# hiropppe/RocAlphaGo

Measured on AMD Instinct MI355X. Metric: positions/sec SL-policy train + MCTS sims/sec (19x19) at 1/2/4/8 MI355X, higher is better.
Workload: dtype bf16; 1 GPU; global_batch=256, per_gpu_batch=256, seq_len=361, parallelism=dp1

## Files before the change

### csrc/hip/conv_wino.hip

```cpp
#include <atomic>

#include "common.h"
#include "conv_host.h"
#include "pack.h"
#include "rag_api.h"

using namespace rag;

namespace {

constexpr int kWK = 32;
constexpr int kWP = 192;
constexpr int kVRows = 224;
constexpr int kRRows = 512;
constexpr int kVSlot = kVRows * kWK;
constexpr int kLoopLds = 4 * kVSlot;
constexpr int kRedU = 14;

template <int WN, int PAIRS> struct WinoGeo;
template <> struct WinoGeo<192, 192> {
  static constexpr int MW = 2, MT = 6, NT = 3, RG = 2;
};
template <> struct WinoGeo<128, 192> {
  static constexpr int MW = 4, MT = 3, NT = 4, RG = 1;
};
template <> struct WinoGeo<192, 96> {
  static constexpr int MW = 2, MT = 3, NT = 3, RG = 1;
};
template <int WN, int PAIRS> struct WinoTile : WinoGeo<WN, PAIRS> {
  using G = WinoGeo<WN, PAIRS>;
  static_assert(G::MW * 16 * G::MT == PAIRS && (8 / G::MW) * 16 * G::NT == WN, "wave tiling");
  static constexpr int EpRow = WN + 8;
  static constexpr int EpImg = 2 * PAIRS * EpRow;
  static constexpr int Lds = kLoopLds > EpImg ? kLoopLds : EpImg;
  static_assert(Lds * 2 <= 160 * 1024, "LDS budget");
};
constexpr int kHalfPairs = 96;

__device__ __forceinline__ int swz4w(int row) { return ((row >> 2) & 1) << 1; }

template <int V> struct IntC {
  static constexpr int value = V;
};

typedef uint32_t u32x4 __attribute__((ext_vector_type(4)));
template <int SGN>
__device__ __forceinline__ bf16x8 vaddsub(const bf16x8& a, const bf16x8& b) {
  const u32x4 ua = __builtin_bit_cast(u32x4, a), ub = __builtin_bit_cast(u32x4, b);
  u32x4 o;
#pragma unroll
  for (int w = 0; w < 4; ++w) {
    const float a0 = __uint_as_float(ua[w] << 16), a1 = __uint_as_float(ua[w] & 0xffff0000u);
    const float b0 = __uint_as_float(ub[w] << 16), b1 = __uint_as_float(ub[w] & 0xffff0000u);
    const bf16x2 r = {(bf16)(SGN > 0 ? a0 + b0 : a0 - b0), (bf16)(SGN > 0 ? a1 + b1 : a1 - b1)};
    o[w] = __builtin_bit_cast(uint32_t, r);
  }
  return __builtin_bit_cast(bf16x8, o);
}
__device__ __forceinline__ bf16x8 vsum(const bf16x8& a, const bf16x8& b) { return vaddsub<1>(a, b); }
__device__ __forceinline__ bf16x8 vdiff(const bf16x8& a, const bf16x8& b) { return vaddsub<-1>(a, b); }
template <int SGN>
__device__ __forceinline__ bf16x8 vaddsub_bn(const bf16x8& a, const bf16x8& b, float cxa,
                                             float cca, float cxb, float ccb) {
  const u32x4 ua = __builtin_bit_cast(u32x4, a), ub = __builtin_bit_cast(u32x4, b);
  u32x4 o;
#pragma unroll
  for (int w = 0; w < 4; ++w) {
    const float a0 = fmaxf(fmaf(cxa, __uint_as_float(ua[w] << 16), cca), 0.f);
    const float a1 = fmaxf(fmaf(cxa, __uint_as_float(ua[w] & 0xffff0000u), cca), 0.f);
    const float b0 = fmaxf(fmaf(cxb, __uint_as_float(ub[w] << 16), ccb), 0.f);
    const float b1 = fmaxf(fmaf(cxb, __uint_as_float(ub[w] & 0xffff0000u), ccb), 0.f);
    const bf16x2 r = {(bf16)(SGN > 0 ? a0 + b0 : a0 - b0), (bf16)(SGN > 0 ? a1 + b1 : a1 - b1)};
    o[w] = __builtin_bit_cast(uint32_t, r);
  }
  return __builtin_bit_cast(bf16x8, o);
}

struct WinoBN {
  const float* coef;
  const bf16* res;
  float* spart;
  const float* smean;
};

template <bool SINGLE, int MT> struct WinoGeom {
  int lane, wm, wn, frow, fq;
  int TJ, PB, RPB;
  int b0, n0, p0;
  long total_rows;
  int vb[SINGLE ? 1 : MT];
  uint32_t uoff;
  int tu0, tu1;
};

__device__ __forceinline__ auto wino_rsrc(const void* p, long bytes) {
  const uint64_t a = reinterpret_cast<uint64_t>(p);
  const uint32_t lo = __builtin_amdgcn_readfirstlane((uint32_t)a);
  const uint32_t hi = __builtin_amdgcn_readfirstlane((uint32_t)(a >> 32));
  const int nb = __builtin_amdgcn_readfirstlane((int)(bytes < 0x7fffffffL ? bytes : 0x7fffffffL));
  return __builtin_amdgcn_make_buffer_rsrc(reinterpret_cast<void*>(((uint64_t)hi << 32) | lo),
                                           (short)0, nb, 0x00020000);
}

template <typename R>
__device__ __forceinline__ uint32_t wino_warm(const R& urs, int NOUT, int KIN) {
  uint32_t warm = 0;
  const int lin = blockIdx.y * gridDim.x + blockIdx.x;
  const int per_xcd = (gridDim.x * gridDim.y + 7) >> 3;
  const uint32_t slice = (uint32_t)((12L * NOUT * KIN * 2 + per_xcd - 1) / per_xcd);
  const uint32_t base = (uint32_t)((lin >> 3) % per_xcd) * slice;
#pragma unroll
  for (int k = 0; k < 4; ++k) {
    const uint32_t off = (uint32_t)(threadIdx.x + k * 512) * 16u;
    const uint32_t o = off < slice ? base + off : 0xfffffff0u;
    warm ^= (uint32_t)__builtin_amdgcn_raw_buffer_load_b32(urs, o, 0, 0);
  }
  return warm;
}

template <int WN, bool SINGLE, int PAIRS>
__device__ __forceinline__ WinoGeom<SINGLE, WinoTile<WN, PAIRS>::MT> wino_geom(int B, int S,
                                                                              int nb) {
  using T = WinoTile<WN, PAIRS>;
  constexpr int kWMT = T::MT;
  constexpr bool HALF = PAIRS == kHalfPairs;
  static_assert(!HALF || SINGLE, "half-board blocks: one board");
  WinoGeom<SINGLE, kWMT> g;
  const int lane = lane_id();
  const int w = wave_id();
  g.lane = lane;
  g.wm = w % T::MW;
  g.wn = w / T::MW;
  g.frow = lane & 15;
  g.fq = lane >> 4;
  const int WI = S + 2, TJ = (S + 1) >> 1;
  const int PB = S * TJ;
  const int VPB = WI * TJ;
  const int RPB = WI * WI;
  g.TJ = TJ;
  g.PB = PB;
  g.RPB = RPB;
  g.b0 = HALF ? (int)(blockIdx.x >> 1) : (int)blockIdx.x * nb;
  g.n0 = blockIdx.y * WN;
  const int p0 = HALF ? (int)(blockIdx.x & 1) * kHalfPairs : 0;
  const int i0 = HALF ? p0 / TJ : 0;
  const int voff = p0 - i0 * TJ;
  g.p0 = p0;
  g.total_rows = (long)B * RPB;
#pragma unroll
  for (int i = 0; i < (SINGLE ? 1 : kWMT); ++i) {
    int m = g.wm * (16 * kWMT) + i * 16 + g.frow;
    if (SINGLE) {
      g.vb[i] = m + voff;
      continue;
    }
    m = m < nb * PB ? m : nb * PB - 1;
    const int bl = m / PB, rem = m - bl * PB;
    const int ii = rem / TJ, t = rem - ii * TJ;
    g.vb[i] = (bl * WI + ii) * TJ + t;
  }
  g.uoff = (uint32_t)((((g.n0 >> 4) + g.wn * T::NT) * 512 + lane * 8) * 2);
  const int NU = HALF ? ((p0 + kHalfPairs - 1) / TJ - i0 + 3) * TJ * 4 : nb * VPB * 4;
  auto unit = [&](int it) {
    const int u = threadIdx.x + it * 512;
    const int v = u >> 2;
    const int bl = v / VPB, rem = v - bl * VPB;
    const int r = rem / TJ, t = rem - r * TJ;
    const int rr = (bl * WI + r + i0) * WI + 2 * t;
    return u < NU ? (v | ((u & 3) << 10) | (rr << 12)) : -1;
  };
  g.tu0 = unit(0);
  g.tu1 = unit(1);
  return g;
}

template <int WN, bool SINGLE, int PAIRS, int BNM, bool CHAIN, typename R>
__device__ __forceinline__ void wino_layer(
    const R& urs, bf16* lds, const WinoGeom<SINGLE, WinoTile<WN, PAIRS>::MT>& g,
    const bf16* __restrict__ X, const float* __restrict__ bias, bf16* __restrict__ Y,
    const bf16* __restrict__ mask, int B, int S, int KIN, int NOUT, int HO, int YC, int relu,
    int HM, int nb, const WinoBN& bn, const bf16* Unext) {
  using T = WinoTile<WN, PAIRS>;
  constexpr int kWMT = T::MT, kWNT = T::NT, kWN = WN, kEpRow = T::EpRow;
  constexpr bool HALF = PAIRS == kHalfPairs;
  static_assert(BNM == 0 || (SINGLE && !HALF && WN == 128), "fused BN: the 128-wide one-board tile");
  static_assert(!CHAIN || (BNM == 0 && !HALF), "chain: plain one- or multi-board blocks");
  float* sred = reinterpret_cast<float*>(lds + T::Lds);
  const int lane = g.lane, wm = g.wm, wn = g.wn, frow = g.frow, fq = g.fq;
  const int TJ = g.TJ, PB = g.PB, RPB = g.RPB, b0 = g.b0, n0 = g.n0, p0 = g.p0;
  const long total_rows = g.total_rows;
  const int tu0 = g.tu0, tu1 = g.tu1;
  const int cchunks = KIN / kWK;
  const int NK = 2 * cchunks;
  int vb[SINGLE ? 1 : kWMT];
#pragma unroll
  for (int i = 0; i < (SINGLE ? 1 : kWMT); ++i) vb[i] = g.vb[i];

  const int NF = NOUT / 16;
  const uint32_t uoff = g.uoff;
  auto wfrag = [&](int tap, int c, int j) {
    const int so = ((tap * cchunks + c) * NF + j) * 1024;
    return __builtin_bit_cast(bf16x8, __builtin_amdgcn_raw_buffer_load_b128(urs, uoff, so, 0));
  };

  float bcx[2][4], bcc[2][4];
  if constexpr (BNM == 1) {
#pragma unroll
    for (int q = 0; q < 2; ++q) {
      const int pk = q ? tu1 : tu0;
      const int v = pk < 0 ? 0 : (pk & 1023);
      const int r = v / TJ, t = v - r * TJ;
      const bool rin = pk >= 0 && r >= 1 && r <= S;
#pragma unroll
      for (int s = 0; s < 4; ++s) {
        const int pc = 2 * t + s;
        const bool in = rin && pc >= 1 && pc <= S;
        bcx[q][s] = in ? bn.coef[pc - 1] : 0.f;
        bcc[q][s] = in ? bn.coef[2 * S + pc - 1] : 0.f;
      }
    }
  }
  const auto xrs = wino_rsrc(X + (long)b0 * RPB * KIN, (total_rows - (long)b0 * RPB) * KIN * 2);
  bf16x8 da0, db0, da1, db1;
  auto op_unit = [&](int o, int& v, int& k8, int& rr) {
    int pk = (o >> 1) ? tu1 : tu0;
    asm volatile("" : "+v"(pk));
    v = pk < 0 ? -1 : (pk & 1023);
    pk = pk < 0 ? 0 : pk;
    k8 = (pk >> 10) & 3;
    rr = pk >> 12;
  };
  auto op_load = [&](auto p1c, int kk, auto oc) {
    constexpr bool P1 = decltype(p1c)::value;
    constexpr int o = decltype(oc)::value, h = o & 1;
    int v, k8, rr;
    op_unit(o, v, k8, rr);
    const int ra = P1 ? 1 : (h ? 3 : 0), rb = P1 ? 2 : (h ? 1 : 2);
    const int so = (kk % cchunks) * kWK * 2;
    const uint32_t o0 = (uint32_t)((rr + ra) * KIN + k8 * 8) * 2u;
    const uint32_t o1 = (uint32_t)((rr + rb) * KIN + k8 * 8) * 2u;
    const bf16x8 a = __builtin_bit_cast(bf16x8, __builtin_amdgcn_raw_buffer_load_b128(xrs, o0, so, 0));
    const bf16x8 b = __builtin_bit_cast(bf16x8, __builtin_amdgcn_raw_buffer_load_b128(xrs, o1, so, 0));
    if constexpr (h) {
      da1 = a;
      db1 = b;
    } else {
      da0 = a;
      db0 = b;
    }
  };
  auto op_store = [&](auto p1c, int kk, auto oc) {
    constexpr bool P1 = decltype(p1c)::value;
    constexpr int o = decltype(oc)::value, h = o & 1;
    int v, k8, rr;
    op_unit(o, v, k8, rr);
    v = v < 0 ? kVRows - 1 : v;
    bf16* vs = lds + (kk & 1) * 2 * kVSlot + h * kVSlot;
    const bf16x8 da = h ? da1 : da0, db = h ? db1 : db0;
    bf16x8 val;
    if constexpr (BNM == 1) {
      constexpr int q = o >> 1, ra = P1 ? 1 : (h ? 3 : 0), rb = P1 ? 2 : (h ? 1 : 2);
      if constexpr (P1 && h)
        val = vaddsub_bn<-1>(db, da, bcx[q][rb], bcc[q][rb], bcx[q][ra], bcc[q][ra]);
      else
        val = vaddsub_bn<P1 ? 1 : -1>(da, db, bcx[q][ra], bcc[q][ra], bcx[q][rb], bcc[q][rb]);
    } else {
      val = P1 ? (h ? vdiff(db, da) : vsum(da, db)) : vdiff(da, db);
    }
    *reinterpret_cast<bf16x8*>(vs + v * kWK + ((k8 ^ swz4w(v)) * 8)) = val;
  };

  f32x4 accA[kWNT][kWMT], accB[kWNT][kWMT];
#pragma unroll
  for (int j = 0; j < kWNT; ++j)
#pragma unroll
    for (int i = 0; i < kWMT; ++i) {
      accA[j][i] = f32x4{0.f, 0.f, 0.f, 0.f};
      accB[j][i] = f32x4{0.f, 0.f, 0.f, 0.f};
    }
  constexpr int kH = kWMT / T::RG;
  bf16x8 xa[kH], wA[kWNT], wB[kWNT];
  auto read_v = [&](int kk, int ky, int set, int h) {
    const bf16* vs = lds + ((kk & 1) * 2 + set) * kVSlot;
    const int sh = ky * TJ;
    if constexpr (SINGLE) {
      int r0 = vb[0];
      asm volatile("" : "+v"(r0));
      r0 += sh + h * kH * 16;
      const int sw0 = (fq ^ swz4w(r0)) * 8;
#pragma unroll
      for (int i = 0; i < kH; ++i)
        xa[i] = *reinterpret_cast<const bf16x8*>(vs + (r0 + i * 16) * kWK + sw0);
    } else {
#pragma unroll
      for (int i = 0; i < kH; ++i) {
        int v = vb[h * kH + i];
        asm volatile("" : "+v"(v));
        const int r = v + sh;
        xa[i] = *reinterpret_cast<const bf16x8*>(vs + r * kWK + ((fq ^ swz4w(r)) * 8));
      }
    }
  };

  uint32_t warm = 0;
  if constexpr (!CHAIN) warm = wino_warm(urs, NOUT, KIN);
#pragma unroll
  for (int j = 0; j < kWNT; ++j) {
    wA[j] = wfrag(1, 0, j);
    wB[j] = wfrag(2, 0, j);
  }
  op_load(IntC<1>{}, 0, IntC<0>{});
  op_store(IntC<1>{}, 0, IntC<0>{});
  op_load(IntC<1>{}, 0, IntC<1>{});
  op_store(IntC<1>{}, 0, IntC<1>{});
  op_load(IntC<1>{}, 0, IntC<2>{});
  op_store(IntC<1>{}, 0, IntC<2>{});
  op_load(IntC<1>{}, 0, IntC<3>{});
  op_store(IntC<1>{}, 0, IntC<3>{});
  if constexpr (!CHAIN) asm volatile("" ::"v"(warm));
  asm volatile("s_waitcnt lgkmcnt(0)" ::: "memory");
  __builtin_amdgcn_s_barrier();
  asm volatile("" ::: "memory");

  auto chunk_phase = [&](int kk, auto curc, auto nxtc) {
    constexpr bool CUR1 = decltype(curc)::value, NXT1 = decltype(nxtc)::value;
#pragma unroll
    for (int ky = 0; ky < 3; ++ky) {
      const bool nxt1 = ky < 2 ? CUR1 : NXT1;
      int nkk = ky < 2 ? kk : kk + 1, nky = ky < 2 ? ky + 1 : 0;
      if (nkk >= NK) {
        nkk = NK - 1;
        nky = 2;
      }
      const int nc = nkk % cchunks;
      const int ntA = nky * 4 + (nxt1 ? 1 : 0), ntB = nky * 4 + (nxt1 ? 2 : 3);
      if (ky == 1) op_store(nxtc, kk + 1, IntC<0>{});
      if (ky == 2) op_store(nxtc, kk + 1, IntC<2>{});
      __builtin_amdgcn_sched_barrier(0);
      if (ky == 0) op_load(nxtc, kk + 1, IntC<0>{});
      if (ky == 1) op_load(nxtc, kk + 1, IntC<2>{});
      __builtin_amdgcn_sched_barrier(0);
#pragma unroll
      for (int h = 0; h < T::RG; ++h) {
        read_v(kk, ky, 0, h);
#pragma unroll
        for (int j = 0; j < kWNT; ++j) {
#pragma unroll
          for (int i = 0; i < kH; ++i)
            accA[j][h * kH + i] = mfma16(wA[j], xa[i], accA[j][h * kH + i]);
          if (h == T::RG - 1) wA[j] = wfrag(ntA, nc, j);
        }
      }
      __builtin_amdgcn_sched_barrier(0);
      if (ky == 1) op_store(nxtc, kk + 1, IntC<1>{});
      if (ky == 2) op_store(nxtc, kk + 1, IntC<3>{});
      __builtin_amdgcn_sched_barrier(0);
      if (ky == 0) op_load(nxtc, kk + 1, IntC<1>{});
      if (ky == 1) op_load(nxtc, kk + 1, IntC<3>{});
      __builtin_amdgcn_sched_barrier(0);
#pragma unroll
      for (int h = 0; h < T::RG; ++h) {
        read_v(kk, ky, 1, h);
#pragma unroll
        for (int j = 0; j < kWNT; ++j) {
#pragma unroll
          for (int i = 0; i < kH; ++i)
            accB[j][h * kH + i] = mfma16(wB[j], xa[i], accB[j][h * kH + i]);
          if (h == T::RG - 1) wB[j] = wfrag(ntB, nc, j);
        }
      }
      __builtin_amdgcn_sched_barrier(0);
    }
    asm volatile("s_waitcnt lgkmcnt(0)" ::: "memory");
    __builtin_amdgcn_s_barrier();
    asm volatile("" ::: "memory");
  };

#pragma unroll 1
  for (int kk = 0; kk < cchunks - 1; ++kk) chunk_phase(kk, IntC<1>{}, IntC<1>{});
  chunk_phase(cchunks - 1, IntC<1>{}, IntC<0>{});
#pragma unroll
  for (int j = 0; j < kWNT; ++j)
#pragma unroll
    for (int i = 0; i < kWMT; ++i) {
      const f32x4 a = accA[j][i], b = accB[j][i];
      accA[j][i] = a + b;
      accB[j][i] = a - b;
    }
#pragma unroll 1
  for (int kk = cchunks; kk < NK; ++kk) chunk_phase(kk, IntC<0>{}, IntC<0>{});

  if constexpr (CHAIN) warm = wino_warm(wino_rsrc(Unext, 12L * NOUT * KIN * 2), NOUT, KIN);
  __syncthreads();
#pragma unroll
  for (int j = 0; j < kWNT; ++j) {
    const int n = wn * (16 * kWNT) + j * 16 + fq * 4;
    float4 bb = {0.f, 0.f, 0.f, 0.f};
    if (bias) bb = *reinterpret_cast<const float4*>(bias + n0 + n);
#pragma unroll
    for (int i = 0; i < kWMT; ++i) {
      const int m = wm * (16 * kWMT) + i * 16 + frow;
      bf16x4 oa, ob;
      const float va[4] = {accA[j][i][0] + bb.x, accA[j][i][1] + bb.y, accA[j][i][2] + bb.z,
                           accA[j][i][3] + bb.w};
      const float vb4[4] = {accB[j][i][0] + bb.x, accB[j][i][1] + bb.y, accB[j][i][2] + bb.z,
                            accB[j][i][3] + bb.w};
#pragma unroll
      for (int r = 0; r < 4; ++r) {
        oa[r] = (bf16)(relu ? fmaxf(va[r], 0.f) : va[r]);
        ob[r] = (bf16)(relu ? fmaxf(vb4[r], 0.f) : vb4[r]);
      }
      *reinterpret_cast<bf16x4*>(lds + (2 * m) * kEpRow + n) = oa;
      *reinterpret_cast<bf16x4*>(lds + (2 * m + 1) * kEpRow + n) = ob;
    }
  }
  if constexpr (CHAIN) asm volatile("" ::"v"(warm));
  __syncthreads();
  if constexpr (BNM != 0) {
    const int S2 = S * S, WO = S + 2 * HO, WMK = S + 2 * HM;
    constexpr int kChunks = kWN / 8;
    const int total = S2 * kChunks, nit = (total + 511) / 512;
    const bool st = bn.spart != nullptr;
    for (int it = 0; it < nit; ++it) {
      const int e = threadIdx.x + it * 512;
      const bool valid = e < total;
      const int pix = valid ? e / kChunks : 0, k8 = (e % kChunks) * 8;
      const int i = pix / S, j = pix - (pix / S) * S;
      float s0 = 0.f, s1 = 0.f;
      if (valid) {
        const int m = i * TJ + (j >> 1);
        bf16x8 v = *reinterpret_cast<const bf16x8*>(lds + (2 * m + (j & 1)) * kEpRow + k8);
        const size_t yo = (size_t)((b0 * WO + i + HO) * WO + j + HO) * YC + n0 + k8;
        if constexpr (BNM == 1) {
          if (bn.res) {
            const bf16x8 r = *reinterpret_cast<const bf16x8*>(bn.res + yo);
#pragma unroll
            for (int q = 0; q < 8; ++q) v[q] = (bf16)((float)v[q] + (float)r[q]);
          }
#pragma unroll
          for (int q = 0; q < 8; ++q) {
            const float f = (float)v[q];
            s0 += f;
            s1 = fmaf(f, f, s1);
          }
        } else {
          const bf16x8 mk = *reinterpret_cast<const bf16x8*>(
              mask + (size_t)((b0 * WMK + i + HM) * WMK + j + HM) * YC + n0 + k8);
          const float cx = bn.coef[j], cc = bn.coef[2 * S + j];
          const float mu = bn.smean ? bn.smean[j] : 0.f;
#pragma unroll
          for (int q = 0; q < 8; ++q) {
            const float xm = (float)mk[q];
            v[q] = fmaf(cx, xm, cc) > 0.f ? v[q] : (bf16)0.f;
            const float d = (float)v[q];
            s0 += d;
            s1 = fmaf(d, xm - mu, s1);
          }
        }
        *reinterpret_cast<bf16x8*>(Y + yo) = v;
      }
      if (st) {
#pragma unroll
        for (int o = kChunks / 2; o > 0; o >>= 1) {
          s0 += __shfl_xor(s0, o, 64);
          s1 += __shfl_xor(s1, o, 64);
        }
        if ((threadIdx.x & (kChunks - 1)) == 0 && valid) {
          atomicAdd(sred + j, s0);
          atomicAdd(sred + 64 + j, s1);
        }
      }
    }
    if (st) {
      __syncthreads();
      if ((int)threadIdx.x < 2 * S) {
        const int q = threadIdx.x / S, c = threadIdx.x - q * S;
        bn.spart[((size_t)blockIdx.x * 2 + q) * S + c] = sred[q * 64 + c];
      }
    }
  } else {
    const int nbl = B - b0 < nb ? B - b0 : nb;
    const int S2 = S * S, WO = S + 2 * HO, WMK = S + 2 * HM;
    constexpr int kChunks = kWN / 8;
    const int pe = p0 + kHalfPairs < PB ? p0 + kHalfPairs : PB;
    const int pixb = HALF ? (p0 / TJ) * S + 2 * (p0 % TJ) : 0;
    const int pixe = HALF ? (pe / TJ) * S + 2 * (pe % TJ) : 0;
    const int total = HALF ? ((pixe < S2 ? pixe : S2) - pixb) * kChunks : nbl * S2 * kChunks;
    for (int e = threadIdx.x; e < total; e += 512) {
      const int pix = e / kChunks + pixb, k8 = (e - (e / kChunks) * kChunks) * 8;
      const int bl = HALF ? 0 : pix / S2, rem = pix - bl * S2;
      const int i = rem / S, j = rem - i * S;
      const int m = bl * PB + i * TJ + (j >> 1) - p0;
      bf16x8 v = *reinterpret_cast<const bf16x8*>(lds + (2 * m + (j & 1)) * kEpRow + k8);
      const int b = b0 + bl;
      if (mask) {
        const bf16x8 mk = *reinterpret_cast<const bf16x8*>(
            mask + (size_t)((b * WMK + i + HM) * WMK + j + HM) * YC + n0 + k8);
#pragma unroll
        for (int q = 0; q < 8; ++q) v[q] = ((float)mk[q] > 0.f) ? v[q] : (bf16)0.f;
      }
      *reinterpret_cast<bf16x8*>(Y + (size_t)((b * WO + i + HO) * WO + j + HO) * YC + n0 + k8) = v;
    }
  }
}

template <int WN, bool SINGLE, int PAIRS = kWP, int BNM = 0>
__global__ void __launch_bounds__(512, 1)
conv_wino_kernel(const bf16* __restrict__ X, const bf16* __restrict__ U,
                 const float* __restrict__ bias, bf16* __restrict__ Y,
                 const bf16* __restrict__ mask, int B, int S, int KIN, int NOUT, int HO, int YC,
                 int relu, int HM, int nb, WgradRed red, WinoBN bn = WinoBN{}) {
  using T = WinoTile<WN, PAIRS>;
  __shared__ __attribute__((aligned(16))) bf16 lds[T::Lds + (BNM ? 256 : 0)];
  if constexpr (BNM != 0) {
    float* sred = reinterpret_cast<float*>(lds + T::Lds);
    if (bn.spart && threadIdx.x < 128) sred[threadIdx.x] = 0.f;
  }
  const auto urs = wino_rsrc(U, 12L * NOUT * KIN * 2);
  const auto g = wino_geom<WN, SINGLE, PAIRS>(B, S, nb);
  wino_layer<WN, SINGLE, PAIRS, BNM, false>(urs, lds, g, X, bias, Y, mask, B, S, KIN, NOUT, HO,
                                            YC, relu, HM, nb, bn, nullptr);
  if (red.ticket) wslab_reduce_dynamic<kRedU>(red, reinterpret_cast<int*>(lds));
}

constexpr int kChainMax = 16;
struct WinoChain {
  bf16* act[kChainMax + 1];
  const bf16* U[kChainMax];
  const float* bias[kChainMax];
  uint32_t relu;
  int L;
};
template <int WN, bool SINGLE>
__global__ void __launch_bounds__(512, 1)
conv_wino_chain_kernel(WinoChain c, int B, int S, int nb) {
  using T = WinoTile<WN, kWP>;
  __shared__ __attribute__((aligned(16))) bf16 lds[T::Lds];
  const auto g = wino_geom<WN, SINGLE, kWP>(B, S, nb);
  const uint32_t warm = wino_warm(wino_rsrc(c.U[0], 12L * WN * WN * 2), WN, WN);
  asm volatile("" ::"v"(warm));
#pragma unroll 1
  for (int l = 0; l < c.L; ++l) {
    const int ln = l + 1 < c.L ? l + 1 : l;
    wino_layer<WN, SINGLE, kWP, 0, true>(wino_rsrc(c.U[l], 12L * WN * WN * 2), lds, g, c.act[l],
                                         c.bias[l], c.act[l + 1], nullptr, B, S, WN, WN, 1, WN,
                                         (int)((c.relu >> l) & 1u), 1, nb, WinoBN{}, c.U[ln]);
    asm volatile("s_waitcnt vmcnt(0) lgkmcnt(0)" ::: "memory");
    __builtin_amdgcn_fence(__ATOMIC_RELEASE, "workgroup");
    __syncthreads();
    __builtin_amdgcn_fence(__ATOMIC_ACQUIRE, "workgroup");
  }
}

__global__ void __launch_bounds__(256) __attribute__((amdgpu_waves_per_eu(4)))
wino_pack_kernel(const int64_t* __restrict__ table, SgdFold sgd) {
  __shared__ float tl[kWinoPackLds];
  wino_pack_block(table, (int)blockIdx.y, (int)blockIdx.x, sgd, tl);
}

struct SgdRest {
  float* p;
  long a0, n0, a1, n1;
};

__global__ void __launch_bounds__(256) __attribute__((amdgpu_waves_per_eu(4)))
pack_step_kernel(const int64_t* __restrict__ wtable, int nwino,
                 const int64_t* __restrict__ ttable, int nrows, int nfull, int max_taps,
                 SgdFold sgd, SgdRest rest) {
  extern __shared__ float lds_dyn[];
  int y = (int)blockIdx.y;
  const int bx = (int)blockIdx.x, gx = (int)gridDim.x;
  const int trows = nfull + (nrows > nfull ? 1 : 0);
  if (y < trows) {
    pack_trunk_block(ttable, y, nrows, nfull, sgd, bx, gx, max_taps, lds_dyn);
    return;
  }
  y -= trows;
  const long n = rest.n0 + rest.n1;
  if (n > 0 && y == 0) {
    for (long i = (long)bx * 256 + threadIdx.x; i < n; i += (long)gx * 256) {
      float* w = rest.p + (i < rest.n0 ? rest.a0 + i : rest.a1 + (i - rest.n0));
      *w = sgd.update(*w, w[sgd.goff]);
    }
    return;
  }
  y -= n > 0 ? 1 : 0;
  if (y < nwino) wino_pack_block(wtable, y, bx, sgd, lds_dyn);
}

int wino_boards_per_block(int S) {
  const int WI = S + 2, TJ = (S + 1) / 2;
  const int PB = S * TJ, VPB = WI * TJ, RPB = WI * WI;
  int nb = kWP / PB;
  if (nb * VPB > kVRows) nb = kVRows / VPB;
  if (nb * RPB + 1 > kRRows) nb = (kRRows - 1) / RPB;
  return nb;
}

int wino_tile(int NOUT, int S) {
  if (NOUT % 192 == 0) return 192;
  if (NOUT == 128 && wino_boards_per_block(S) == 1) return 128;
  return 0;
}

}

RAG_API int rag_conv_wino_ok(int S, int HI, int KIN, int NOUT, int KS) {
  return KS == 3 && HI == 1 && KIN % kWK == 0 && KIN >= kWK && S >= 2 &&
         wino_boards_per_block(S) >= 1 && wino_tile(NOUT, S) > 0;
}

static bool wino_half_ok(int S, int NOUT) {
  const int TJ = (S + 1) / 2;
  return NOUT % 192 == 0 && wino_boards_per_block(S) == 1 && S * TJ > kHalfPairs;
}
static int wino_cus() {
  static std::atomic<int> cus{0};
  int n = cus.load(std::memory_order_relaxed);
  if (!n) {
    int dev = 0;
    if (hipGetDevice(&dev) != hipSuccess ||
        hipDeviceGetAttribute(&n, hipDeviceAttributeMultiprocessorCount, dev) != hipSuccess)
      return 0;
    cus.store(n, std::memory_order_relaxed);
  }
  return n;
}
static int wino_mode(int B, int S, int KIN, int NOUT) {
  if (!rag_conv_wino_ok(S, 1, KIN, NOUT, 3) || B <= 0 || wino_boards_per_block(S) != 1) return 0;
  const int cus = wino_cus();
  if (!cus) return 0;
  auto fills = [&](long blocks) {
    const long waves = (blocks + cus - 1) / cus;
    return blocks * 8 >= waves * cus * 7;
  };
  const long full = (long)B * (NOUT / wino_tile(NOUT, S));
  const bool half = wino_half_ok(S, NOUT);
  if (full <= cus) return half && 2 * full <= cus ? 2 : 1;
  if (fills(full)) return 1;
  if (half && fills(2 * full)) return 2;
  return 0;
}
RAG_API int rag_conv_wino_mode(int B, int S, int KIN, int NOUT) {
  return wino_mode(B, S, KIN, NOUT);
}

int rag_conv_wino_launch(const void* X, const void* W, const float* bias, void* Y,
                         const void* mask, int B, int S, int KIN, int NOUT, int HO, int YC,
                         int relu, int HM, hipStream_t stream, const WgradRed* red, int half) {
  if (!rag_conv_wino_ok(S, 1, KIN, NOUT, 3) || YC < NOUT || B <= 0) return -1;
  const int nb = wino_boards_per_block(S);
  WgradRed r{};
  if (red) r = *red;
  const int wt = wino_tile(NOUT, S);
  const dim3 grid((B + nb - 1) / nb, NOUT / wt);
  if (wt == 192 && ((half && wino_half_ok(S, NOUT)) || wino_mode(B, S, KIN, NOUT) == 2))
    conv_wino_kernel<192, true, kHalfPairs><<<dim3(2 * B, NOUT / wt), 512, 0, stream>>>(
        (const bf16*)X, (const bf16*)W, bias, (bf16*)Y, (const bf16*)mask, B, S, KIN, NOUT, HO,
        YC, relu, HM, 1, r);
  else if (wt == 128)
    conv_wino_kernel<128, true><<<grid, 512, 0, stream>>>((const bf16*)X, (const bf16*)W, bias,
                                                          (bf16*)Y, (const bf16*)mask, B, S, KIN,
                                                          NOUT, HO, YC, relu, HM, nb, r);
  else if (nb == 1)
    conv_wino_kernel<192, true><<<grid, 512, 0, stream>>>((const bf16*)X, (const bf16*)W, bias,
                                                          (bf16*)Y, (const bf16*)mask, B, S, KIN,
                                                          NOUT, HO, YC, relu, HM, nb, r);
  else
    conv_wino_kernel<192, false><<<grid, 512, 0, stream>>>((const bf16*)X, (const bf16*)W, bias,
                                                           (bf16*)Y, (const bf16*)mask, B, S, KIN,
                                                           NOUT, HO, YC, relu, HM, nb, r);
  return (int)hipGetLastError();
}

static bool wino_bn_ok(int B, int S, int KIN, int NOUT) {
  return NOUT == 128 && KIN == 128 && S <= 64 && wino_tile(NOUT, S) == 128 &&
         wino_mode(B, S, KIN, NOUT) == 1;
}
RAG_API int rag_conv_wino_bn_ok(int B, int S, int KIN, int NOUT) {
  return wino_bn_ok(B, S, KIN, NOUT);
}

int rag_conv_wino_bn_launch(const void* X, const void* W, const float* bias, void* Y,
                            const void* mask, const void* res, int B, int S, int KIN, int NOUT,
                            int HO, int YC, int relu, int HM, hipStream_t stream,
                            const WgradRed* red, const float* coef, const float* mcoef,
                            float* spart, const float* smean) {
  if (!wino_bn_ok(B, S, KIN, NOUT) || YC < NOUT || (coef != nullptr) == (mcoef != nullptr) ||
      (mcoef && (!mask || res)) || (smean && !mcoef))
    return -5;
  WgradRed r{};
  if (red) r = *red;
  if (coef)
    conv_wino_kernel<128, true, kWP, 1><<<B, 512, 0, stream>>>(
        (const bf16*)X, (const bf16*)W, bias, (bf16*)Y, nullptr, B, S, KIN, NOUT, HO, YC, relu,
        HM, 1, r, WinoBN{coef, (const bf16*)res, spart, nullptr});
  else
    conv_wino_kernel<128, true, kWP, 2><<<B, 512, 0, stream>>>(
        (const bf16*)X, (const bf16*)W, bias, (bf16*)Y, (const bf16*)mask, B, S, KIN, NOUT, HO,
        YC, relu, HM, 1, r, WinoBN{mcoef, nullptr, spart, smean});
  return (int)hipGetLastError();
}

RAG_API int rag_conv_wino_chain(const int64_t* table, int L, int B, int S, hipStream_t stream,
                                int any_batch) {
  constexpr int kF = 7;
  if (!table || L < 1 || L > kChainMax || B <= 0) return -1;
  const int C = (int)table[5];
  if (!rag_conv_wino_ok(S, 1, C, C, 3) || wino_tile(C, S) != C) return -1;
  if (!any_batch && wino_mode(B, S, C, C) != 1) return -1;
  WinoChain c{};
  c.L = L;
  for (int l = 0; l < L; ++l) {
    const int64_t* r = table + (size_t)l * kF;
    if (r[5] != C || r[6] != C || !r[0] || !r[1] || !r[3]) return -1;
    if (l > 0 && r[0] != table[(size_t)(l - 1) * kF + 3]) return -1;
    c.act[l] = reinterpret_cast<bf16*>(r[0]);
    c.act[l + 1] = reinterpret_cast<bf16*>(r[3]);
    c.U[l] = reinterpret_cast<const bf16*>(r[1]);
    c.bias[l] = reinterpret_cast<const float*>(r[2]);
    if (r[4]) c.relu |= 1u << l;
  }
  const int64_t bytes = (int64_t)B * (S + 2) * (S + 2) * C * 2;
  for (int i = 0; i <= L; ++i)
    for (int j = 0; j < i; ++j) {
      const int64_t d = reinterpret_cast<int64_t>(c.act[i]) - reinterpret_cast<int64_t>(c.act[j]);
      if ((d < 0 ? -d : d) < bytes) return -1;
    }
  const int nb = wino_boards_per_block(S);
  const dim3 grid((B + nb - 1) / nb);
  if (C == 128)
    conv_wino_chain_kernel<128, true><<<grid, 512, 0, stream>>>(c, B, S, nb);
  else if (nb == 1)
    conv_wino_chain_kernel<192, true><<<grid, 512, 0, stream>>>(c, B, S, nb);
  else
    conv_wino_chain_kernel<192, false><<<grid, 512, 0, stream>>>(c, B, S, nb);
  return (int)hipGetLastError();
}

RAG_API int rag_wino_pack(const int64_t* table, int nlayers, int max_tiles, hipStream_t stream,
                          int64_t goff, float lr, float wd, int sgd_on) {
  if (nlayers <= 0 || max_tiles <= 0) return -1;
  const dim3 grid((unsigned)(8 * max_tiles), (unsigned)nlayers);
  wino_pack_kernel<<<grid, 256, 0, stream>>>(table, SgdFold{(long)goff, lr, wd, sgd_on});
  return (int)hipGetLastError();
}

RAG_API int rag_pack_step(const int64_t* wtable, int nwino, const int64_t* ttable, int nrows,
                          int nfull, int max_taps, int width, hipStream_t stream, int64_t goff,
                          float lr, float wd, int sgd_on, float* flat, int64_t a0, int64_t n0,
                          int64_t a1, int64_t n1) {
  if (nwino < 0 || nrows < 0 || nfull < 0 || nfull > nrows || width <= 0 || max_taps < 1 ||
      max_taps > kPTaps || n0 < 0 || n1 < 0 || (nwino > 0 && !wtable) || (nrows > 0 && !ttable))
    return -1;
  const bool rest = sgd_on && n0 + n1 > 0;
  if (rest && !flat) return -1;
  const int trows = nfull + (nrows > nfull ? 1 : 0);
  const int rows = nwino + trows + (rest ? 1 : 0);
  if (rows == 0) return 0;
  const int l1 = kWinoPackLds, l2 = pack_trunk_lds(max_taps);
  const size_t lds = (size_t)(nfull > 0 && l2 > l1 ? l2 : l1) * sizeof(float);
  const SgdRest r{flat, (long)a0, rest ? (long)n0 : 0L, (long)a1, rest ? (long)n1 : 0L};
  pack_step_kernel<<<dim3((unsigned)width, (unsigned)rows), 256, lds, stream>>>(
      wtable, nwino, ttable, nrows, nfull, max_taps, SgdFold{(long)goff, lr, wd, sgd_on}, r);
  return (int)hipGetLastError();
}
```

Baseline: 124,300 positions/s.

## Restructure Winograd input-transform pipeline with XOR-flipped LDS ring and precomputed offsets

Reworks the Winograd conv main loop. Per-unit global and LDS offsets are now computed once in the geometry setup instead of being decoded every chunk, and LDS double-buffering switches to an XOR flip bit rather than kk-based slot arithmetic. The P1 pass computes sum and difference together in one fused helper, so one load pair feeds two stores. Half-board blocks now use a single load unit, and a host check keeps that path only when its unit count fits in 512 threads. This cuts address arithmetic and VALU work in the hot loop, at the cost of more persistent registers and a larger LDS footprint from the flip offset.

Result: faster. 127,500 positions/s, median of 6 (+2.5%).

```diff
diff --git a/csrc/hip/conv_wino.hip b/csrc/hip/conv_wino.hip
--- a/csrc/hip/conv_wino.hip
+++ b/csrc/hip/conv_wino.hip
@@ -14,7 +14,9 @@
 constexpr int kVRows = 224;
 constexpr int kRRows = 512;
 constexpr int kVSlot = kVRows * kWK;
-constexpr int kLoopLds = 4 * kVSlot;
+constexpr int kVFlip = 32768;
+constexpr int kLoopLds = kVFlip / 2 + 2 * kVSlot;
+static_assert(2 * kVSlot * 2 <= kVFlip, "V ring: a buffer below the flip bit");
 constexpr int kRedU = 14;
 
 template <int WN, int PAIRS> struct WinoGeo;
@@ -57,8 +59,21 @@
   }
   return __builtin_bit_cast(bf16x8, o);
 }
-__device__ __forceinline__ bf16x8 vsum(const bf16x8& a, const bf16x8& b) { return vaddsub<1>(a, b); }
 __device__ __forceinline__ bf16x8 vdiff(const bf16x8& a, const bf16x8& b) { return vaddsub<-1>(a, b); }
+__device__ __forceinline__ void vsumdiff(const bf16x8& a, const bf16x8& b, bf16x8& s, bf16x8& d) {
+  const u32x4 ua = __builtin_bit_cast(u32x4, a), ub = __builtin_bit_cast(u32x4, b);
+  u32x4 os, od;
+#pragma unroll
+  for (int w = 0; w < 4; ++w) {
+    const float a0 = __uint_as_float(ua[w] << 16), a1 = __uint_as_float(ua[w] & 0xffff0000u);
+    const float b0 = __uint_as_float(ub[w] << 16), b1 = __uint_as_float(ub[w] & 0xffff0000u);
+    const bf16x2 rs = {(bf16)(a0 + b0), (bf16)(a1 + b1)}, rd = {(bf16)(b0 - a0), (bf16)(b1 - a1)};
+    os[w] = __builtin_bit_cast(uint32_t, rs);
+    od[w] = __builtin_bit_cast(uint32_t, rd);
+  }
+  s = __builtin_bit_cast(bf16x8, os);
+  d = __builtin_bit_cast(bf16x8, od);
+}
 template <int SGN>
 __device__ __forceinline__ bf16x8 vaddsub_bn(const bf16x8& a, const bf16x8& b, float cxa,
                                              float cca, float cxb, float ccb) {
@@ -74,6 +89,24 @@
     o[w] = __builtin_bit_cast(uint32_t, r);
   }
   return __builtin_bit_cast(bf16x8, o);
+}
+
+__device__ __forceinline__ void vsumdiff_bn(const bf16x8& a, const bf16x8& b, float cxa, float cca,
+                                            float cxb, float ccb, bf16x8& s, bf16x8& d) {
+  const u32x4 ua = __builtin_bit_cast(u32x4, a), ub = __builtin_bit_cast(u32x4, b);
+  u32x4 os, od;
+#pragma unroll
+  for (int w = 0; w < 4; ++w) {
+    const float a0 = fmaxf(fmaf(cxa, __uint_as_float(ua[w] << 16), cca), 0.f);
+    const float a1 = fmaxf(fmaf(cxa, __uint_as_float(ua[w] & 0xffff0000u), cca), 0.f);
+    const float b0 = fmaxf(fmaf(cxb, __uint_as_float(ub[w] << 16), ccb), 0.f);
+    const float b1 = fmaxf(fmaf(cxb, __uint_as_float(ub[w] & 0xffff0000u), ccb), 0.f);
+    const bf16x2 rs = {(bf16)(a0 + b0), (bf16)(a1 + b1)}, rd = {(bf16)(b0 - a0), (bf16)(b1 - a1)};
+    os[w] = __builtin_bit_cast(uint32_t, rs);
+    od[w] = __builtin_bit_cast(uint32_t, rd);
+  }
+  s = __builtin_bit_cast(bf16x8, os);
+  d = __builtin_bit_cast(bf16x8, od);
 }
 
 struct WinoBN {
@@ -91,6 +124,9 @@
   int vb[SINGLE ? 1 : MT];
   uint32_t uoff;
   int tu0, tu1;
+  uint32_t ru[2];
+  int su[2];
+  int rv[3];
 };
 
 __device__ __forceinline__ auto wino_rsrc(const void* p, long bytes) {
@@ -120,7 +156,7 @@
 
 template <int WN, bool SINGLE, int PAIRS>
 __device__ __forceinline__ WinoGeom<SINGLE, WinoTile<WN, PAIRS>::MT> wino_geom(int B, int S,
-                                                                              int nb) {
+                                                                              int nb, int KIN) {
   using T = WinoTile<WN, PAIRS>;
   constexpr int kWMT = T::MT;
   constexpr bool HALF = PAIRS == kHalfPairs;
@@ -160,7 +196,8 @@
     g.vb[i] = (bl * WI + ii) * TJ + t;
   }
   g.uoff = (uint32_t)((((g.n0 >> 4) + g.wn * T::NT) * 512 + lane * 8) * 2);
-  const int NU = HALF ? ((p0 + kHalfPairs - 1) / TJ - i0 + 3) * TJ * 4 : nb * VPB * 4;
+  const int pe = p0 + kHalfPairs < PB ? p0 + kHalfPairs : PB;
+  const int NU = HALF ? ((pe - 1) / TJ - i0 + 3) * TJ * 4 : nb * VPB * 4;
   auto unit = [&](int it) {
     const int u = threadIdx.x + it * 512;
     const int v = u >> 2;
@@ -170,19 +207,33 @@
     return u < NU ? (v | ((u & 3) << 10) | (rr << 12)) : -1;
   };
   g.tu0 = unit(0);
-  g.tu1 = unit(1);
+  g.tu1 = HALF ? -1 : unit(1);
+#pragma unroll
+  for (int u = 0; u < 2; ++u) {
+    const int pk = u ? g.tu1 : g.tu0;
+    const int v = pk < 0 ? kVRows - 1 : (pk & 1023);
+    const int k8 = pk < 0 ? 0 : (pk >> 10) & 3, rr = pk < 0 ? 0 : pk >> 12;
+    g.ru[u] = (uint32_t)(rr * KIN + k8 * 8) * 2u;
+    g.su[u] = (v * kWK + ((k8 ^ swz4w(v)) * 8)) * 2;
+  }
+#pragma unroll
+  for (int ky = 0; ky < 3; ++ky) {
+    const int r = g.vb[0] + ky * TJ;
+    g.rv[ky] = (r * kWK + ((g.fq ^ swz4w(r)) * 8)) * 2;
+  }
   return g;
 }
 
 template <int WN, bool SINGLE, int PAIRS, int BNM, bool CHAIN, typename R>
 __device__ __forceinline__ void wino_layer(
-    const R& urs, bf16* lds, const WinoGeom<SINGLE, WinoTile<WN, PAIRS>::MT>& g,
+    const R& urs, bf16* lds, WinoGeom<SINGLE, WinoTile<WN, PAIRS>::MT>& g,
     const bf16* __restrict__ X, const float* __restrict__ bias, bf16* __restrict__ Y,
     const bf16* __restrict__ mask, int B, int S, int KIN, int NOUT, int HO, int YC, int relu,
     int HM, int nb, const WinoBN& bn, const bf16* Unext) {
   using T = WinoTile<WN, PAIRS>;
   constexpr int kWMT = T::MT, kWNT = T::NT, kWN = WN, kEpRow = T::EpRow;
   constexpr bool HALF = PAIRS == kHalfPairs;
+  constexpr int kUnits = HALF ? 1 : 2;
   static_assert(BNM == 0 || (SINGLE && !HALF && WN == 128), "fused BN: the 128-wide one-board tile");
   static_assert(!CHAIN || (BNM == 0 && !HALF), "chain: plain one- or multi-board blocks");
   float* sred = reinterpret_cast<float*>(lds + T::Lds);
@@ -191,10 +242,10 @@
   const long total_rows = g.total_rows;
   const int tu0 = g.tu0, tu1 = g.tu1;
   const int cchunks = KIN / kWK;
-  const int NK = 2 * cchunks;
   int vb[SINGLE ? 1 : kWMT];
 #pragma unroll
   for (int i = 0; i < (SINGLE ? 1 : kWMT); ++i) vb[i] = g.vb[i];
+  int vpar = 0;
 
   const int NF = NOUT / 16;
   const uint32_t uoff = g.uoff;
@@ -222,25 +273,21 @@
   }
   const auto xrs = wino_rsrc(X + (long)b0 * RPB * KIN, (total_rows - (long)b0 * RPB) * KIN * 2);
   bf16x8 da0, db0, da1, db1;
-  auto op_unit = [&](int o, int& v, int& k8, int& rr) {
-    int pk = (o >> 1) ? tu1 : tu0;
-    asm volatile("" : "+v"(pk));
-    v = pk < 0 ? -1 : (pk & 1023);
-    pk = pk < 0 ? 0 : pk;
-    k8 = (pk >> 10) & 3;
-    rr = pk >> 12;
-  };
-  auto op_load = [&](auto p1c, int kk, auto oc) {
+  auto op_load = [&](auto p1c, int c, auto oc) {
     constexpr bool P1 = decltype(p1c)::value;
-    constexpr int o = decltype(oc)::value, h = o & 1;
-    int v, k8, rr;
-    op_unit(o, v, k8, rr);
-    const int ra = P1 ? 1 : (h ? 3 : 0), rb = P1 ? 2 : (h ? 1 : 2);
-    const int so = (kk % cchunks) * kWK * 2;
-    const uint32_t o0 = (uint32_t)((rr + ra) * KIN + k8 * 8) * 2u;
-    const uint32_t o1 = (uint32_t)((rr + rb) * KIN + k8 * 8) * 2u;
-    const bf16x8 a = __builtin_bit_cast(bf16x8, __builtin_amdgcn_raw_buffer_load_b128(xrs, o0, so, 0));
-    const bf16x8 b = __builtin_bit_cast(bf16x8, __builtin_amdgcn_raw_buffer_load_b128(xrs, o1, so, 0));
+    constexpr int o = decltype(oc)::value, u = P1 ? o : o >> 1, h = P1 ? o : o & 1;
+    constexpr int ra = P1 ? 1 : (h ? 3 : 0), rb = P1 ? 2 : (h ? 1 : 2);
+    const int so = c * kWK * 2;
+    uint32_t roa = g.ru[u];
+    if constexpr (ra == 3) {
+      asm volatile("" : "+v"(roa));
+      roa += 3u * (uint32_t)KIN * 2u;
+    }
+    const int soa = so + (ra == 3 ? 0 : ra * KIN * 2);
+    const bf16x8 a = __builtin_bit_cast(
+        bf16x8, __builtin_amdgcn_raw_buffer_load_b128(xrs, roa, soa, 0));
+    const bf16x8 b = __builtin_bit_cast(
+        bf16x8, __builtin_amdgcn_raw_buffer_load_b128(xrs, g.ru[u], so + rb * KIN * 2, 0));
     if constexpr (h) {
       da1 = a;
       db1 = b;
@@ -249,25 +296,40 @@
       db0 = b;
     }
   };
-  auto op_store = [&](auto p1c, int kk, auto oc) {
+  auto op_store = [&](auto p1c, auto oc) {
     constexpr bool P1 = decltype(p1c)::value;
-    constexpr int o = decltype(oc)::value, h = o & 1;
-    int v, k8, rr;
-    op_unit(o, v, k8, rr);
-    v = v < 0 ? kVRows - 1 : v;
-    bf16* vs = lds + (kk & 1) * 2 * kVSlot + h * kVSlot;
+    constexpr int o = decltype(oc)::value, u = P1 ? o : o >> 1, h = P1 ? o : o & 1;
+    constexpr int ra = P1 ? 1 : (h ? 3 : 0), rb = P1 ? 2 : (h ? 1 : 2);
+    char* vs = reinterpret_cast<char*>(lds) + g.su[u];
     const bf16x8 da = h ? da1 : da0, db = h ? db1 : db0;
-    bf16x8 val;
-    if constexpr (BNM == 1) {
-      constexpr int q = o >> 1, ra = P1 ? 1 : (h ? 3 : 0), rb = P1 ? 2 : (h ? 1 : 2);
-      if constexpr (P1 && h)
-        val = vaddsub_bn<-1>(db, da, bcx[q][rb], bcc[q][rb], bcx[q][ra], bcc[q][ra]);
+    if constexpr (P1) {
+      bf16x8 vs1, vs2;
+      if constexpr (BNM == 1)
+        vsumdiff_bn(da, db, bcx[u][ra], bcc[u][ra], bcx[u][rb], bcc[u][rb], vs1, vs2);
       else
-        val = vaddsub_bn<P1 ? 1 : -1>(da, db, bcx[q][ra], bcc[q][ra], bcx[q][rb], bcc[q][rb]);
+        vsumdiff(da, db, vs1, vs2);
+      *reinterpret_cast<bf16x8*>(vs) = vs1;
+      *reinterpret_cast<bf16x8*>(vs + kVSlot * 2) = vs2;
     } else {
-      val = P1 ? (h ? vdiff(db, da) : vsum(da, db)) : vdiff(da, db);
-    }
-    *reinterpret_cast<bf16x8*>(vs + v * kWK + ((k8 ^ swz4w(v)) * 8)) = val;
+      bf16x8 val;
+      if constexpr (BNM == 1)
+        val = vaddsub_bn<-1>(da, db, bcx[u][ra], bcc[u][ra], bcx[u][rb], bcc[u][rb]);
+      else
+        val = vdiff(da, db);
+      *reinterpret_cast<bf16x8*>(vs + h * kVSlot * 2) = val;
+    }
+  };
+  auto flip_su = [&]() {
+#pragma unroll
+    for (int u = 0; u < kUnits; ++u) g.su[u] ^= kVFlip;
+  };
+  auto flip_rv = [&]() {
+    if constexpr (SINGLE) {
+#pragma unroll
+      for (int ky = 0; ky < 3; ++ky) g.rv[ky] ^= kVFlip;
+    } else {
+      vpar ^= kVFlip;
+    }
   };
 
   f32x4 accA[kWNT][kWMT], accB[kWNT][kWMT];
@@ -280,18 +342,17 @@
     }
   constexpr int kH = kWMT / T::RG;
   bf16x8 xa[kH], wA[kWNT], wB[kWNT];
-  auto read_v = [&](int kk, int ky, int set, int h) {
-    const bf16* vs = lds + ((kk & 1) * 2 + set) * kVSlot;
-    const int sh = ky * TJ;
+  auto read_v = [&](int ky, int set, int h) {
     if constexpr (SINGLE) {
-      int r0 = vb[0];
-      asm volatile("" : "+v"(r0));
-      r0 += sh + h * kH * 16;
-      const int sw0 = (fq ^ swz4w(r0)) * 8;
+      const char* vs = reinterpret_cast<const char*>(lds) + g.rv[ky];
 #pragma unroll
       for (int i = 0; i < kH; ++i)
-        xa[i] = *reinterpret_cast<const bf16x8*>(vs + (r0 + i * 16) * kWK + sw0);
+        xa[i] = *reinterpret_cast<const bf16x8*>(
+            vs + (set * kVSlot + (h * kH + i) * 16 * kWK) * 2);
     } else {
+      const bf16* vs = reinterpret_cast<const bf16*>(reinterpret_cast<const char*>(lds) + vpar) +
+                       set * kVSlot;
+      const int sh = ky * TJ;
 #pragma unroll
       for (int i = 0; i < kH; ++i) {
         int v = vb[h * kH + i];
@@ -310,39 +371,43 @@
     wB[j] = wfrag(2, 0, j);
   }
   op_load(IntC<1>{}, 0, IntC<0>{});
-  op_store(IntC<1>{}, 0, IntC<0>{});
-  op_load(IntC<1>{}, 0, IntC<1>{});
-  op_store(IntC<1>{}, 0, IntC<1>{});
-  op_load(IntC<1>{}, 0, IntC<2>{});
-  op_store(IntC<1>{}, 0, IntC<2>{});
-  op_load(IntC<1>{}, 0, IntC<3>{});
-  op_store(IntC<1>{}, 0, IntC<3>{});
+  op_store(IntC<1>{}, IntC<0>{});
+  if constexpr (kUnits == 2) {
+    op_load(IntC<1>{}, 0, IntC<1>{});
+    op_store(IntC<1>{}, IntC<1>{});
+  }
+  flip_su();
   if constexpr (!CHAIN) asm volatile("" ::"v"(warm));
   asm volatile("s_waitcnt lgkmcnt(0)" ::: "memory");
   __builtin_amdgcn_s_barrier();
   asm volatile("" ::: "memory");
 
-  auto chunk_phase = [&](int kk, auto curc, auto nxtc) {
+  auto slot_store = [&](auto nxtc, auto tc) {
+    constexpr bool NXT1 = decltype(nxtc)::value;
+    constexpr int o = decltype(tc)::value - 2;
+    if constexpr (o >= 0 && o < (NXT1 ? 1 : 2) * kUnits) op_store(nxtc, IntC<o>{});
+  };
+  auto slot_load = [&](auto nxtc, int cn, auto tc) {
+    constexpr bool NXT1 = decltype(nxtc)::value;
+    constexpr int o = decltype(tc)::value;
+    if constexpr (o < (NXT1 ? 1 : 2) * kUnits) op_load(nxtc, cn, IntC<o>{});
+  };
+
+  auto chunk_phase = [&](int c, int cn, bool last, auto curc, auto nxtc) {
     constexpr bool CUR1 = decltype(curc)::value, NXT1 = decltype(nxtc)::value;
-#pragma unroll
-    for (int ky = 0; ky < 3; ++ky) {
+    auto step = [&](auto kyc) {
+      constexpr int ky = decltype(kyc)::value;
       const bool nxt1 = ky < 2 ? CUR1 : NXT1;
-      int nkk = ky < 2 ? kk : kk + 1, nky = ky < 2 ? ky + 1 : 0;
-      if (nkk >= NK) {
-        nkk = NK - 1;
-        nky = 2;
-      }
-      const int nc = nkk % cchunks;
+      const int nc = ky < 2 || last ? c : cn;
+      const int nky = ky < 2 ? ky + 1 : (last ? 2 : 0);
       const int ntA = nky * 4 + (nxt1 ? 1 : 0), ntB = nky * 4 + (nxt1 ? 2 : 3);
-      if (ky == 1) op_store(nxtc, kk + 1, IntC<0>{});
-      if (ky == 2) op_store(nxtc, kk + 1, IntC<2>{});
+      slot_store(nxtc, IntC<2 * ky>{});
       __builtin_amdgcn_sched_barrier(0);
-      if (ky == 0) op_load(nxtc, kk + 1, IntC<0>{});
-      if (ky == 1) op_load(nxtc, kk + 1, IntC<2>{});
+      slot_load(nxtc, cn, IntC<2 * ky>{});
       __builtin_amdgcn_sched_barrier(0);
 #pragma unroll
       for (int h = 0; h < T::RG; ++h) {
-        read_v(kk, ky, 0, h);
+        read_v(ky, 0, h);
 #pragma unroll
         for (int j = 0; j < kWNT; ++j) {
 #pragma unroll
@@ -352,15 +417,13 @@
         }
       }
       __builtin_amdgcn_sched_barrier(0);
-      if (ky == 1) op_store(nxtc, kk + 1, IntC<1>{});
-      if (ky == 2) op_store(nxtc, kk + 1, IntC<3>{});
+      slot_store(nxtc, IntC<2 * ky + 1>{});
       __builtin_amdgcn_sched_barrier(0);
-      if (ky == 0) op_load(nxtc, kk + 1, IntC<1>{});
-      if (ky == 1) op_load(nxtc, kk + 1, IntC<3>{});
+      slot_load(nxtc, cn, IntC<2 * ky + 1>{});
       __builtin_amdgcn_sched_barrier(0);
 #pragma unroll
       for (int h = 0; h < T::RG; ++h) {
-        read_v(kk, ky, 1, h);
+        read_v(ky, 1, h);
 #pragma unroll
         for (int j = 0; j < kWNT; ++j) {
 #pragma unroll
@@ -370,15 +433,20 @@
         }
       }
       __builtin_amdgcn_sched_barrier(0);
-    }
+    };
+    step(IntC<0>{});
+    step(IntC<1>{});
+    step(IntC<2>{});
     asm volatile("s_waitcnt lgkmcnt(0)" ::: "memory");
     __builtin_amdgcn_s_barrier();
     asm volatile("" ::: "memory");
+    flip_su();
+    flip_rv();
   };
 
 #pragma unroll 1
-  for (int kk = 0; kk < cchunks - 1; ++kk) chunk_phase(kk, IntC<1>{}, IntC<1>{});
-  chunk_phase(cchunks - 1, IntC<1>{}, IntC<0>{});
+  for (int c = 0; c < cchunks - 1; ++c) chunk_phase(c, c + 1, false, IntC<1>{}, IntC<1>{});
+  chunk_phase(cchunks - 1, 0, false, IntC<1>{}, IntC<0>{});
 #pragma unroll
   for (int j = 0; j < kWNT; ++j)
 #pragma unroll
@@ -388,7 +456,9 @@
       accB[j][i] = a - b;
     }
 #pragma unroll 1
-  for (int kk = cchunks; kk < NK; ++kk) chunk_phase(kk, IntC<0>{}, IntC<0>{});
+  for (int c = 0; c < cchunks; ++c)
+    chunk_phase(c, c + 1 < cchunks ? c + 1 : 0, c + 1 == cchunks, IntC<0>{}, IntC<0>{});
+  flip_su();
 
   if constexpr (CHAIN) warm = wino_warm(wino_rsrc(Unext, 12L * NOUT * KIN * 2), NOUT, KIN);
   __syncthreads();
@@ -517,7 +587,7 @@
     if (bn.spart && threadIdx.x < 128) sred[threadIdx.x] = 0.f;
   }
   const auto urs = wino_rsrc(U, 12L * NOUT * KIN * 2);
-  const auto g = wino_geom<WN, SINGLE, PAIRS>(B, S, nb);
+  auto g = wino_geom<WN, SINGLE, PAIRS>(B, S, nb, KIN);
   wino_layer<WN, SINGLE, PAIRS, BNM, false>(urs, lds, g, X, bias, Y, mask, B, S, KIN, NOUT, HO,
                                             YC, relu, HM, nb, bn, nullptr);
   if (red.ticket) wslab_reduce_dynamic<kRedU>(red, reinterpret_cast<int*>(lds));
@@ -536,7 +606,7 @@
 conv_wino_chain_kernel(WinoChain c, int B, int S, int nb) {
   using T = WinoTile<WN, kWP>;
   __shared__ __attribute__((aligned(16))) bf16 lds[T::Lds];
-  const auto g = wino_geom<WN, SINGLE, kWP>(B, S, nb);
+  auto g = wino_geom<WN, SINGLE, kWP>(B, S, nb, WN);
   const uint32_t warm = wino_warm(wino_rsrc(c.U[0], 12L * WN * WN * 2), WN, WN);
   asm volatile("" ::"v"(warm));
 #pragma unroll 1
@@ -610,9 +680,20 @@
          wino_boards_per_block(S) >= 1 && wino_tile(NOUT, S) > 0;
 }
 
+static int wino_half_units(int S) {
+  const int TJ = (S + 1) / 2, PB = S * TJ;
+  int most = 0;
+  for (int p0 = 0; p0 < PB; p0 += kHalfPairs) {
+    const int pe = p0 + kHalfPairs < PB ? p0 + kHalfPairs : PB;
+    const int n = ((pe - 1) / TJ - p0 / TJ + 3) * TJ * 4;
+    most = n > most ? n : most;
+  }
+  return most;
+}
 static bool wino_half_ok(int S, int NOUT) {
   const int TJ = (S + 1) / 2;
-  return NOUT % 192 == 0 && wino_boards_per_block(S) == 1 && S * TJ > kHalfPairs;
+  return NOUT % 192 == 0 && wino_boards_per_block(S) == 1 && S * TJ > kHalfPairs &&
+         wino_half_units(S) <= 512;
 }
 static int wino_cus() {
   static std::atomic<int> cus{0};
```
